# zzmuxi/simian-spacemonkey

Measured on AMD Instinct MI355X. Metric: Msamples/s + fps, 512^3 VGH vol @1024^2 x 512 steps, higher is better.
Workload: dtype f32

## Files before the change

simian-spacemonkey_amd/csrc/smk_api.hip:

```cpp
#include <math.h>
#include <stdio.h>
#include <string.h>

#include <algorithm>

#include "smk_device.h"

static std::string g_create_err;

#include <condition_variable>
#include <mutex>
#include <thread>
namespace {
struct HostPool {
  std::vector<std::thread> workers;
  std::mutex m, use;
  std::condition_variable cv, done_cv;
  const std::function<void(int)> *job = nullptr;
  int njobs = 0, next = 0, pending = 0;
  unsigned long long gen = 0;
  bool quit = false;
  explicit HostPool(int n) {
    for (int i = 0; i < n; ++i)
      workers.emplace_back([this] {
// ... 875 lines not shown
  for (int r = 0; r < c->nranks; ++r) {
    int key = 0;
    for (int bit = 0; bit < nbits; ++bit)
      if (((r >> bit) & 1) != nearbit[bit % 3]) key |= 1 << bit;
    keyed.push_back({key, r});
  }
  std::sort(keyed.begin(), keyed.end());
  for (int r = 0; r < c->nranks; ++r) order[r] = keyed[r].second;
}

extern "C" int smk_shard_order(smk_ctx *c, int *order) {
  if (!c || !order) return 1;
  if (!c->have_volume || !c->have_camera) FAIL(c, "smk_shard_order: volume and camera must be set");
  double inv[16];
  smk_inverse_affine(inv, c->mv);
  double e[3];
  for (int a = 0; a < 3; ++a) e[a] = inv[12 + a] * c->N[a] / c->fsize[a] - 0.5;
  smk_bsp_order(c, e, order);
  return 0;
}


extern "C" int smk_set_option(smk_ctx *c, const char *key, int value) {
  if (!c || !key) return 1;
  if (!strcmp(key, "kernel")) c->opt_kernel = value;
  else if (!strcmp(key, "slab_T")) c->slab.opt_T = value & 0xff;
  else if (!strcmp(key, "inject_slab_status")) c->opt_inject_status = value;
  else if (!strcmp(key, "slab_fly")) c->slab.opt_fly = value < 0 ? 0 : (value > 63 ? 63 : value);
  else if (!strcmp(key, "slab_ns")) c->slab.opt_ns = value < 0 ? 0 : (value > 63 ? 63 : value);
  else if (!strcmp(key, "tile")) c->slab.opt_tile = value;
  else if (!strcmp(key, "shadow_march")) c->opt_shadow_march = value ? 1 : 0;
  else if (!strcmp(key, "shadow_fused")) c->opt_lockstep = value ? (c->opt_lockstep | 256) : (c->opt_lockstep & ~256);
  else if (!strcmp(key, "slab_split")) c->slab.opt_split = value < 0 ? 0 : (value > 8 ? 8 : value);
  else if (!strcmp(key, "cols_shape")) c->cols.opt_shape = value & 0xff;
  else if (!strcmp(key, "cols_ns")) c->cols.opt_ns = value & 0xff;
  else if (!strcmp(key, "cols_chunk")) c->cols.opt_chunk = value & 0xfff;
  else if (!strcmp(key, "cols_wstep")) c->cols.opt_wstep = value & 7;
  else if (!strcmp(key, "cols_counts")) c->cols.want_counts = value ? 1 : 0;
  else if (!strcmp(key, "cols_fill")) { c->cols.opt_fill = value; smk_cols_drop_layouts(&c->cols); }
  else if (!strcmp(key, "cols_take_min")) c->cols.opt_take_min = value;
  else if (!strcmp(key, "cols_take_wait")) c->cols.opt_take_wait = value;
  else if (!strcmp(key, "cols_fly")) c->cols.opt_fly = value;
  else if (!strcmp(key, "bricks")) {
    c->opt_bricks = value ? 1 : 0;
    c->tf_dirty = true;
    c->bricks3_dirty = true;
  }
  else if (!strcmp(key, "wave_w")) {
    if (!(value == 1 || value == 2 || value == 4 || value == 8 || value == 16 || value == 32 || value == 64)) FAIL(c, "smk_set_option: wave_w must be a power of two <= 64");
    c->opt_wave_w = value;
  } else if (!strcmp(key, "blk_w")) {
    if (!(value == 1 || value == 2 || value == 4)) FAIL(c, "smk_set_option: blk_w must be 1, 2 or 4");
    c->opt_blk_w = value;
  } else if (!strcmp(key, "lockstep")) c->opt_lockstep = value;
  else if (!strcmp(key, "tf_raw")) {
    c->opt_tf_raw = value;
    c->tf_dirty = true;
  }
  else if (!strcmp(key, "halo")) {
    if (c->have_volume) FAIL(c, "smk_set_option: halo must be set before smk_upload_volume");
    if (value < 1) FAIL(c, "smk_set_option: halo must be >= 1");
    c->halo = value;
  } else
    FAIL(c, "smk_set_option: unknown key '%s'", key);
  return 0;
}
// ... 50 lines not shown
    return count_on_device(c, [&](unsigned long long *d) { return smk_launch_shadow_count_light(P, sc, olo, ohi, d, c->stream); }, value);
  }
  if (!strcmp(name, "slab_status")) {
    HIPCHK(c, hipDeviceSynchronize());
    *value = c->slab.h_status ? (((volatile int *)c->slab.h_status)[c->slab.status_slot] & 0xff) : 0;
    return 0;
  }
  if (!strcmp(name, "slab_failures")) {
    long long n = c->slab_failures;
    if (c->slab.h_status)
      for (int k = 0; k < SMK_STATUS_RING; ++k) n += ((volatile int *)c->slab.h_status)[k] != 0;
    *value = (double)n;
    return 0;
  }
  if (!strcmp(name, "slab_streamed_fraction")) {
    *value = 1.0;
    const int nt = c->slab.ticks_n_last;
    if (c->last_kernel == 2 && c->slab.d_ticks && nt > 0) {
      std::vector<unsigned> h((size_t)2 * nt);
      if (read_back(c, h.data(), c->slab.d_ticks + nt, h.size())) return 1;
      double st = 0, pl = 0;
      for (int t = 0; t < nt; ++t) {
        st += h[t];
        pl += h[(size_t)nt + t];
      }
      if (pl > 0) *value = st / pl;
    }
    return 0;
  }
  if (!strcmp(name, "slab_tile_ms_max") || !strcmp(name, "slab_tile_ms_sum")) {
    *value = 0.0;
    const int nt = c->slab.ticks_n_last;
    if (c->last_kernel == 2 && c->slab.d_ticks && nt > 0) {
      std::vector<unsigned> h((size_t)nt);
      if (read_back(c, h.data(), c->slab.d_ticks, h.size())) return 1;
      double mx = 0, sum = 0;
      for (int t = 0; t < nt; ++t) {
        const double k = t < (int)c->slab.ksplit_last.size() ? std::max<int>(c->slab.ksplit_last[t], 1) : 1;
        mx = std::max(mx, (double)h[t] / k);
        sum += h[t];
      }
      *value = (name[13] == 'm' ? mx : sum) * 1e-5;
    }
    return 0;
  }
  if (!strncmp(name, "cols_", 5)) return smk_cols_stat(c, name, value);
  if (!strcmp(name, "slab_split_tiles")) { *value = c->slab.nsplit_last; return 0; }
  if (!strcmp(name, "slab_workgroups")) { *value = c->slab.nblocks_last; return 0; }
  if (!strcmp(name, "slab_retries")) { *value = (double)c->slab_retries; return 0; }
  if (!strcmp(name, "clip_slice_pass")) { *value = c->clip_slice_pass; return 0; }
  FAIL(c, "smk_get_stat: unknown name '%s'", name);
}

extern "C" int smk_get_trace(smk_ctx *c, unsigned *out, int cap_records, int *nrecords) {
  if (!c || !nrecords) return 1;
  HIPCHK(c, hipSetDevice(c->device));
  if (!(c->opt_lockstep & 32)) {
    const int nt = c->last_kernel == 2 && c->slab.d_ticks ? c->slab.ticks_n_last : 0;
    *nrecords = nt;
    if (out && nt > 0) {
      std::vector<unsigned> h((size_t)nt * 5);
      if (read_back(c, h.data(), c->slab.d_ticks, h.size())) return 1;
      for (int t = 0; t < std::min(cap_records, nt); ++t) {
        unsigned *r = out + (size_t)t * 8;
        r[0] = h[(size_t)3 * nt + t];
        r[1] = h[(size_t)3 * nt + t] ? r[0] + h[t] : 0u;
        r[2] = h[(size_t)4 * nt + t] & 0xff00u;
        r[3] = (h[(size_t)4 * nt + t] & 0xfu) | ((unsigned)t << 8) | (h[(size_t)2 * nt + t] << 20);
        r[4] = r[5] = r[6] = r[7] = 0;
      }
    }
    return 0;
  }
  *nrecords = c->slab.d_trace ? c->slab.trace_n : 0;
  if (out && *nrecords > 0 && read_back(c, out, c->slab.d_trace, (size_t)std::min(cap_records, *nrecords) * 8)) return 1;
  return 0;
}

extern "C" int smk_count_samples(smk_ctx *c, double *in_volume) {
  if (!c || !in_volume) return 1;
  HIPCHK(c, hipSetDevice(c->device));
  RenderParams P;
  if (smk_build_params(c, P, c->stream)) return 1;
  smk_shadowcoef sc;
  if (c->shadow_on && c->tf_mode != 0 && !P.pert_on && !c->region_on && smk_shadow_setup(c, P, sc, nullptr, nullptr)) return 1;
  return count_on_device(c, [&](unsigned long long *d) { return smk_launch_count_inside(P, d, c->stream); }, in_volume);
}

void smk_region_box(const smk_ctx *c, const int g0[3], const int g1[3], float lo[3], float hi[3], int top[3]) {
  for (int a = 0; a < 3; ++a) {
    lo[a] = (float)g0[a] - 0.5f;
    hi[a] = (float)g1[a] - 0.5f;
    top[a] = g1[a] == c->N[a];
  }
  if (c->clip_axis >= 1 && c->clip_axis <= 6) {
    const int a = (c->clip_axis - 1) / 2;
    const float fs = c->fsize[a];
    const float cp = c->clip_vpos[a] > 0.0f ? (c->clip_vpos[a] < fs ? c->clip_vpos[a] : fs) : 0.0f;
    const float face = (float)((double)cp / (double)fs * (double)c->N[a] - 0.5);
// ... 357 lines not shown
```

simian-spacemonkey_amd/csrc/smk_internal.h:

```cpp
#pragma once
#include <hip/hip_runtime.h>
#include <stdint.h>

#include <map>
#include <string>
#include <vector>

#include "../../include/smk.h"

#define SMK_MAX_RANKS 8
#define SMK_TIMING_RING 64
#define SMK_BRICK_LOG2 3
#define SMK_SHADOW_BOX_EPS 0.0009765625f
#define SMK_TUNE_SETTLE 6
#define SMK_STATUS_RING 8

#define HIPCHK(ctx, call)                                                              \
  do {                                                                                 \
    hipError_t e_ = (call);                                                            \
    if (e_ != hipSuccess) {                                                            \
      char b_[512];                                                                    \
      snprintf(b_, sizeof b_, "%s failed: %s (%s:%d)", #call, hipGetErrorString(e_), __FILE__, __LINE__); \
      (ctx)->err = b_;                                                                 \
      return 1;                                                                        \
// ... 91 lines not shown
  std::vector<int2> order_host;
  struct Scan {
    std::vector<unsigned char> key;
    double v[4] = {0, 0, 0, 0};
    std::vector<int> work;
  } scan[4];
  unsigned scan_next = 0;
  std::vector<unsigned char> shape_key;
  int shape_choice = -1, shape_age = 0, shape_chunks = 0;
  std::vector<int> plan_work;
  std::vector<unsigned char> plan_cuts;
  std::vector<int2> plan_order;
  int plan_slots = 0;
  unsigned *d_ticks = nullptr, *h_ticks = nullptr;
  int ticks_cap = 0, ticks_pending_n = 0, ticks_age = 0, ticks_adopted = 0;
  int ticks_n_last = 0;
  bool ticks_pending = false;
  long long ticks_pending_sig = 0, ticks_good_sig = -1;
  hipEvent_t ticks_ev = nullptr;
  std::vector<unsigned> ticks_good;
  void *d_seg = nullptr;
  size_t seg_cap = 0;
  int opt_split = 0;
  int opt_tile = 0, opt_T = 0, opt_fly = 0, opt_ns = 0;
  bool ticks_stale = false;
  int nsplit_last = 0, nblocks_last = 0;
  std::vector<unsigned char> ksplit_last;
  unsigned *d_pticks = nullptr, *h_pticks = nullptr;
  std::vector<unsigned> pticks_good;
  std::vector<unsigned char> cuts, cuts_pending, cuts_good;
  int cuts_split = -1;
  long long cuts_sig = -1;
  bool recut = true, cuts_engaged = false, merge_warm = false;
  unsigned *d_trace = nullptr;
  int trace_cap = 0, trace_n = 0;
};

struct ColLayout {
  void *d = nullptr;
  size_t bytes = 0;
  int CW = 0, CH = 0, ncu = 0, ncv = 0, Du = 0, Dv = 0, Ds = 0, slice_bytes = 0, vb = 0;
  const void *src = nullptr;
};
struct ColsAux {
  ColLayout lay[3];
  void *d_layers = nullptr;
  size_t layers_cap = 0;
  void *d_masks = nullptr;
  size_t masks_cap = 0;
  bool masks_dirty = true;
  int mask_words_last = 0;
  unsigned *d_ticks = nullptr;
  int ticks_cap = 0, njobs_last = 0;
  unsigned long long *d_counts = nullptr;
  int want_counts = 0;
  int opt_shape = 0, opt_ns = 0, opt_chunk = 0, opt_wstep = 0;
  int opt_fill = 0, opt_take_min = 0, opt_take_wait = 0, opt_fly = 0;
  int builds = 0;
  int cw_last = 0, ch_last = 0, nslots_last = 0, shape_last = 0;
  double last_stream_bytes = 0;
  hipEvent_t frame_ev0 = nullptr;
  int status_tag = 0;
};
void smk_cols_free(ColsAux *aux);
void smk_cols_drop_layouts(ColsAux *aux);

// ... 240 lines not shown
```

simian-spacemonkey_amd/csrc/smk_slab.hip:

```cpp
#include <math.h>
#include <stdio.h>
#include <stdlib.h>
#include <string.h>

#include <algorithm>
#include <functional>
#include <type_traits>

#include "smk_device.h"
#include "smk_slab.h"

#define SLAB_DONE 0x3fffffff
constexpr int SLAB_POLL_SLEEP = 2;

template <int DT>
struct VoxT;
template <>
struct VoxT<0> {
  typedef uint2 type;
};
template <>
struct VoxT<1> {
  typedef float4 type;
};
// ... 93 lines not shown
  __builtin_memcpy(&lo, tb + off, 8);
  __builtin_memcpy(&hi, tb + (off + (unsigned)ss * 4u), 8);
  o.a = lo.x;
  o.b = lo.y;
  o.c = hi.x;
  o.d = hi.y;
  return o;
}
__device__ __forceinline__ float slab_tex_chan(const SlabTexel4 &x, int k) {
  return smk_lerp(smk_lerp(smk_ub(x.a, k), smk_ub(x.b, k), x.fs), smk_lerp(smk_ub(x.c, k), smk_ub(x.d, k), x.fs), x.ft) * SMK_INV255;
}

template <int DT, int SH, int PERM, int NW, int NL, bool DIAG, int TF = 1, bool BR = true, bool SHD = false, bool OCC = false>
__global__ __launch_bounds__((NW + NL) * 64, ((NW + NL) == 9) ? 6 : ((NW + NL) == 5 || (NW + NL) == 10) ? 5 : ((NW + NL) == 11 ? 3 : (NW + NL) == 12 ? 6 : 4)) void smk_k_slab(const RenderParams P, const SlabParams Q) {
  constexpr int UPV = DT == 0 ? 2 : 1;
  constexpr int VB = DT == 0 ? 8 : 16;
  constexpr int VBL = DT == 0 ? 3 : 4;
  constexpr int NTH = (NW + NL) * 64;
  constexpr bool BIG = slab_big(NW, NL);
  constexpr bool EARLY = BIG;
  constexpr bool FIFO = BIG;
  constexpr int NLG = slab_loader_groups(NW, NL);
  constexpr int LPG = NL / NLG;
  constexpr int QSTEP = NLG;
  extern __shared__ __align__(16) unsigned char smem[];
  SlabEnt *wtab = reinterpret_cast<SlabEnt *>(smem + (size_t)Q.nslots * Q.slot_bytes);
  int *ctl = reinterpret_cast<int *>(smem + (((size_t)Q.nslots * Q.slot_bytes + (size_t)Q.Ds * sizeof(SlabEnt) + 15) & ~(size_t)15));
  float *ah = reinterpret_cast<float *>(ctl + 8 + 32);
  const uint32_t *occ = reinterpret_cast<const uint32_t *>(ah + (Q.use_ah ? P.sv : 0));

  const int2 oent = Q.order[blockIdx.x];
  const int ocode = oent.x;
  if (ocode < 0) return;
  const int tile = ocode & 0xfffff, seg = (ocode >> 20) & 63, nseg = max((ocode >> 26) & 31, 1);
  const int cut_lo = oent.y & 255, cut_hi = (oent.y >> 8) & 255;
  const bool flags = BR && Q.bricks != nullptr;
  const bool tracing = DIAG && Q.trace != nullptr && (P.lockstep & 32);
  const unsigned trace_t0 = (unsigned)__builtin_amdgcn_s_memrealtime();
  const int ty = tile / P.ntx, tx = tile - ty * P.ntx;

  const int tid = threadIdx.x;
  const int lane = tid & 63;
  const int wave = __builtin_amdgcn_readfirstlane(tid >> 6);
  const bool is_loader = wave >= NW;
  const int lid = wave - NW;
  const int wpr = Q.tw >> 3;
  const int i = tx * Q.tw + (wave % wpr) * 8 + (lane & 7);
  const int j = ty * Q.th + (wave / wpr) * 8 + (lane >> 3);
  const bool live = !is_loader && i < P.W && j < P.H;

  const smk_raycoef &rc = P.rc;
  const float px = __fmaf_rn((float)i + 0.5f, rc.pxs, rc.pxl);
  const float py = __fmaf_rn((float)j + 0.5f, rc.pys, rc.pyl);
  float A[3], B[3], tauA, dtau;
  const bool ray_ok = smk_ray_AB_t<SHD>(P, px, py, A, B, tauA, dtau);
  float tenter = 0.0f, texit = (float)(rc.nplanes - 1);
  bool empty = rc.nplanes <= 0 || !live || !ray_ok;
#pragma unroll
  for (int a = 0; a < 3; ++a) {
    if (fabsf(B[a]) > 1e-20f) {
      float inv = 1.0f / B[a];
      float t1 = (P.lo[a] - SMK_RANGE_EPS - A[a]) * inv, t2 = (P.hi[a] + SMK_RANGE_EPS - A[a]) * inv;
      tenter = fmaxf(tenter, fminf(t1, t2) - 2.0f);
      texit = fminf(texit, fmaxf(t1, t2) + 2.0f);
    } else if (!(A[a] >= P.lo[a] && A[a] <= P.hi[a])) {
      empty = true;
    }
  }
  if (P.cplane_on) {
    const float c0 = __fmaf_rn(A[0], P.cplane[0], __fmaf_rn(A[1], P.cplane[1], __fmaf_rn(A[2], P.cplane[2], P.cplane[3])));
    const float c1 = __fmaf_rn(B[0], P.cplane[0], __fmaf_rn(B[1], P.cplane[1], B[2] * P.cplane[2]));
    if (fabsf(c1) > 1e-20f) {
      const float tz = -c0 / c1;
      if (c1 > 0.0f) tenter = fmaxf(tenter, tz - 2.0f);
      else texit = fminf(texit, tz + 2.0f);
    } else if (!(c0 >= 0.0f)) {
      empty = true;
    }
  }
  if (SHD && ray_ok) {
    if (fabsf(dtau) > 1e-30f) {
      const float tz = -tauA / dtau;
// ... 868 lines not shown
            car_i = base_slice_c(m, car_sc);
            pb = __mul24(psgn, car_i) + poff;
          } else pb = SLAB_DONE;
        }
        if (count) {
          n_it += 1.f;
          n_act += (float)__popcll(__ballot(act));
          n_in += (float)__popcll(__ballot(work));
          n_hit += (float)__popcll(__ballot(d_hit));
          n_anyhit += __any(d_hit) ? 1.f : 0.f;
          n_work += __any(work) ? 1.f : 0.f;
          n_own += __any(work && d_own) ? 1.f : 0.f;
        }
        }
      }
      if (lane == 0) lds_st(&ctl[8 + wave], SLAB_DONE);
      if (tracing && lane == 0) atomicAdd(Q.trace + 8 * (size_t)blockIdx.x + 7, (unsigned)n_it);
      if (count && lane == 0) {
        atomicAdd(&Q.diag[0], n_it);
        atomicAdd(&Q.diag[1], n_act);
        atomicAdd(&Q.diag[2], n_in);
        atomicAdd(&Q.diag[3], n_hit);
        atomicAdd(&Q.diag[8], n_anyhit);
        atomicAdd(&Q.diag[14], n_work);
        atomicAdd(&Q.diag[15], n_own);
        atomicAdd(&Q.diag[9], n_lead);
        atomicAdd(&Q.diag[10], n_waits);
        atomicAdd(&Q.diag[11], n_wstep);
        atomicAdd(&Q.diag[12], (float)max(npos - min(pos, npos), 0) / (float)max(npos, 1));
        atomicAdd(&Q.diag[13], 1.0f);
      }
    }
  }
  if (live) {
    size_t o = (size_t)j * P.W + i;
    float4 *outp = seg == 0 ? P.out : Q.seg_out + (size_t)(seg - 1) * ((size_t)P.W * P.H);
    outp[o] = make_float4(C0, C1, C2, C3);
    if (P.depth != nullptr && C3 == 0.0f) P.depth[o] = __int_as_float(0x7f800000);
  }
  if (npos > 0) {
    __syncthreads();
    if (tid == 0 && ctl[3]) *(volatile int *)Q.status = Q.status_tag | ctl[3];
  }
  if (tid == 0 && Q.tile_ticks && nseg > 1) {
    const unsigned dur = max((unsigned)__builtin_amdgcn_s_memrealtime() - trace_t0, 1u);
    if (Q.piece_ticks) Q.piece_ticks[(size_t)tile * 8 + seg] = dur;
    atomicAdd(&Q.tile_ticks[tile], dur);
    atomicAdd(&Q.tile_ticks[Q.ntiles + tile], npos > 0 ? (unsigned)max(min(max(min(min(ctl[4], ctl[5]), min(ctl[6], ctl[7])), 0), npos + 1) - ctl[2], 0) : 0u);
    atomicAdd(&Q.tile_ticks[2 * Q.ntiles + tile], npos > 0 ? (unsigned)(npos + 1) : 0u);
  } else if (tid == 0 && Q.tile_ticks) {
    Q.tile_ticks[tile] = max((unsigned)__builtin_amdgcn_s_memrealtime() - trace_t0, 1u);
    Q.tile_ticks[Q.ntiles + tile] = npos > 0 ? (unsigned)max(min(max(min(min(ctl[4], ctl[5]), min(ctl[6], ctl[7])), 0), npos + 1) - ctl[2], 0) : 0u;
    Q.tile_ticks[2 * Q.ntiles + tile] = npos > 0 ? (unsigned)(npos + 1) : 0u;
    Q.tile_ticks[3 * Q.ntiles + tile] = trace_t0;
    Q.tile_ticks[4 * Q.ntiles + tile] = (__builtin_amdgcn_s_getreg((31 << 11) | 4) & 0xff00u) | (__builtin_amdgcn_s_getreg((31 << 11) | 20) & 0xfu);
  }
  if (tracing && tid == 0) {
    unsigned *t = Q.trace + 8 * (size_t)blockIdx.x;
    if (phases) {
      t[4] = ph1;
      t[5] = ph2;
      t[6] = ph3;
    }
    t[0] = trace_t0;
    t[1] = (unsigned)__builtin_amdgcn_s_memrealtime();
    t[2] = __builtin_amdgcn_s_getreg((31 << 11) | 4);
    t[3] = (__builtin_amdgcn_s_getreg((31 << 11) | 20) & 0xf) | ((unsigned)tile << 8) | ((unsigned)max(npos, 0) << 20);
  }
}


#ifndef SLAB_PART
#define SLAB_PART 0
#endif
#if SLAB_PART == 0
__global__ __launch_bounds__(256) void smk_k_slab_merge(const int2 *list, int tw, int th, int ntx, int W, int H, const float4 *seg_out, float4 *out, int use_max) {
  const int code = list[blockIdx.x].x;
  const int tile = code & 0xfffff, nseg = code >> 20;
  const int ty = tile / ntx, tx = tile - ty * ntx;
  const size_t npix = (size_t)W * H;
  for (int p = threadIdx.x; p < tw * th; p += blockDim.x) {
    const int i = tx * tw + p % tw, j = ty * th + p / tw;
    if (i >= W || j >= H) continue;
    const size_t o = (size_t)j * W + i;
    float4 C = out[o];
    for (int k = 1; k < nseg; ++k) {
      const float4 sgm = seg_out[(size_t)(k - 1) * npix + o];
      if (use_max) {
        C = make_float4(fmaxf(C.x, sgm.x), fmaxf(C.y, sgm.y), fmaxf(C.z, sgm.z), fmaxf(C.w, sgm.w));
      } else {
        const float w = 1.0f - C.w;
        C.x = __fmaf_rn(w, sgm.x, C.x);
        C.y = __fmaf_rn(w, sgm.y, C.y);
        C.z = __fmaf_rn(w, sgm.z, C.z);
        C.w = __fmaf_rn(w, sgm.w, C.w);
      }
    }
    out[o] = C;
  }
}
// ... 130 lines not shown
```

simian-spacemonkey_amd/csrc/smk_slab_plan.hip:

```cpp
#include <math.h>
#include <stdio.h>
#include <stdlib.h>
#include <string.h>
#include <time.h>

#include <algorithm>
#include <vector>

#include "smk_slab.h"

void host_ray_at(const RenderParams &P, double px, double py, double A[3], double B[3]) {
  const smk_raycoef &rc = P.rc;
  if (!P.sh.on) {
    for (int a = 0; a < 3; ++a) {
      A[a] = px * rc.Ax[a] + py * rc.Ay[a] + rc.Ac[a];
      B[a] = px * rc.Bx[a] + py * rc.By[a] + rc.Bc[a];
    }
    return;
  }
  const SmkShadowRays &sh = P.sh;
  const double nD = px * sh.nDx + py * sh.nDy + sh.nDc, tauA = sh.numA / nD, dtau = sh.dB / nD;
  for (int a = 0; a < 3; ++a) {
    const double D = px * sh.Dx[a] + py * sh.Dy[a] + sh.Dc[a];
    A[a] = sh.Ec[a] + tauA * D;
// ... 530 lines not shown
    if (aux->h_pticks) (void)hipHostFree(aux->h_pticks);
    aux->d_ticks = aux->h_ticks = aux->d_pticks = aux->h_pticks = nullptr;
    aux->ticks_cap = 0;
    hipError_t e = hipMalloc((void **)&aux->d_ticks, (size_t)nt * 20);
    if (e == hipSuccess) e = hipMemset(aux->d_ticks, 0, (size_t)nt * 20);
    if (e == hipSuccess) e = hipHostMalloc((void **)&aux->h_ticks, (size_t)nt * 4, hipHostMallocDefault);
    if (e == hipSuccess) e = hipMalloc((void **)&aux->d_pticks, (size_t)nt * 32);
    if (e == hipSuccess) e = hipMemset(aux->d_pticks, 0, (size_t)nt * 32);
    if (e == hipSuccess) e = hipHostMalloc((void **)&aux->h_pticks, (size_t)nt * 32, hipHostMallocDefault);
    if (e != hipSuccess) return e;
    aux->ticks_cap = nt;
  }
  if (!aux->ticks_ev) {
    hipError_t e = hipEventCreateWithFlags(&aux->ticks_ev, hipEventDisableTiming);
    if (e != hipSuccess) return e;
  }
  Q.tile_ticks = aux->d_ticks;
  Q.piece_ticks = aux->d_pticks;
  Q.ntiles = nt;
  aux->ticks_n_last = nt;
  return hipSuccess;
}

void smk_slab_forget_measurements(SlabAux *aux) {
  aux->ticks_good.clear();
  aux->ticks_good_sig = -1;
  aux->ticks_adopted = 0;
  aux->ticks_stale = aux->ticks_pending;
  aux->pticks_good.clear();
  aux->cuts_good.clear();
  aux->cuts.clear();
  aux->cuts_sig = -1;
  aux->cuts_engaged = false;
  aux->recut = true;
}

void smk_slab_free(SlabAux *aux) {
  for (void *p : {(void *)aux->d_diag, (void *)aux->d_order, (void *)aux->d_pticks, aux->d_seg, (void *)aux->d_trace, (void *)aux->d_ticks})
    if (p) (void)hipFree(p);
  for (void *p : {(void *)aux->h_status, (void *)aux->h_pticks, (void *)aux->h_ticks, (void *)aux->h_order[0], (void *)aux->h_order[1],
                  (void *)aux->h_order[2], (void *)aux->h_order[3]})
    if (p) (void)hipHostFree(p);
  for (hipEvent_t e : {aux->order_ev[0], aux->order_ev[1], aux->order_ev[2], aux->order_ev[3], aux->ticks_ev})
    if (e) (void)hipEventDestroy(e);
}

static void slab_cut_segments(SlabAux *aux, const std::vector<int> &work, int nt, long long tsig, int opt_split, bool big) {
  const bool measured = aux->ticks_good_sig == tsig && (int)aux->ticks_good.size() == nt;
  if ((int)aux->cuts.size() != nt * 10 || aux->cuts_split != opt_split || aux->cuts_sig != tsig) {
    aux->cuts.assign((size_t)nt * 10, 0);
    for (int t = 0; t < nt; ++t) { aux->cuts[(size_t)t * 10] = 1; aux->cuts[(size_t)t * 10 + 2] = 255; }
    aux->cuts_split = opt_split;
    aux->cuts_sig = tsig;
    aux->recut = true;
  }
  if (aux->recut) {
    aux->recut = false;
    auto equal_cuts = [&](int t, int K) {
      unsigned char *c = &aux->cuts[(size_t)t * 10];
      c[0] = (unsigned char)K;
      for (int k = 0; k <= K; ++k) c[1 + k] = (unsigned char)(255 * k / K);
    };
    if (opt_split >= 2) {
      for (int t = 0; t < nt; ++t) equal_cuts(t, std::min(opt_split, 8));
    } else if (opt_split == 0 && measured) {
      long long total = 0;
      for (int t = 0; t < nt; ++t) total += work[t];
      const double wg_slots = 256.0 * (big ? 1 : 2);
      const double mean_load = (double)total / wg_slots;
      double longest_tile = 0;
      for (int t = 0; t < nt; ++t) longest_tile = std::max(longest_tile, (double)work[t]);
      const double piece = std::max(0.75 * mean_load, 6000.0);
      bool big_frame = mean_load >= 5000.0 && longest_tile > 1.5 * mean_load;
      if (aux->cuts_engaged && mean_load >= 5000.0 && longest_tile > 1.2 * mean_load) big_frame = true;
      aux->cuts_engaged = big_frame;
      const bool have_pieces = (int)aux->pticks_good.size() == nt * 8 && (int)aux->cuts_good.size() == nt * 10;
      for (int t = 0; t < nt; ++t) {
        unsigned char *c = &aux->cuts[(size_t)t * 10];
        int Kw = (big_frame && (double)work[t] > 1.25 * piece) ? (int)std::min(8.0, ceil((double)work[t] / piece)) : 1;
        if (big_frame && c[0] >= 2 && Kw >= 1 && abs(Kw - (int)c[0]) <= 1 && (double)work[t] > piece) Kw = c[0];
        if (Kw == 1) { equal_cuts(t, 1); continue; }
        const unsigned char *g = have_pieces ? &aux->cuts_good[(size_t)t * 10] : nullptr;
        const int Kg = g ? g[0] : 1;
        if (!g || Kg < 2) {
          if (c[0] != Kw) equal_cuts(t, Kw);
          continue;
        }
        double d[8], tot = 0, longest = 0;
        for (int k = 0; k < Kg; ++k) {
          d[k] = std::max(1.0, (double)aux->pticks_good[(size_t)t * 8 + k] - 1300.0);
          tot += d[k];
          longest = std::max(longest, d[k]);
        }
        const bool same = !memcmp(g, c, 10);
        if (same && Kg == Kw && longest <= 1.3 * tot / Kg) continue;
        unsigned char nc[10] = {(unsigned char)Kw, 0};
        int k = 0;
        double acc = 0;
        for (int j = 1; j < Kw; ++j) {
          const double want = tot * j / Kw;
          while (k < Kg - 1 && acc + d[k] < want) acc += d[k++];
          const double f = d[k] > 0 ? (want - acc) / d[k] : 0.5;
          int x = (int)lround(g[1 + k] + f * (g[2 + k] - g[1 + k]));
          x = std::max(x, (int)nc[j] + 1);
          x = std::min(x, 255 - (Kw - j));
          nc[1 + j] = (unsigned char)x;
        }
        nc[1 + Kw] = 255;
        memcpy(c, nc, 10);
      }
    } else {
      for (int t = 0; t < nt; ++t) equal_cuts(t, 1);
    }
  }
}

static void slab_schedule(const RenderParams &P, SlabAux *aux, const std::vector<int> &work, int slots, std::vector<int2> &order) {
  const int nt = P.ntx * P.nty;
  if (aux->plan_slots == slots && aux->plan_work == work && aux->plan_cuts == aux->cuts && !aux->plan_order.empty()) {
    order = aux->plan_order;
    return;
  }
  std::vector<unsigned char> ksplit((size_t)nt, 1);
  for (int t = 0; t < nt; ++t) ksplit[t] = aux->cuts[(size_t)t * 10];
  auto piece_weight = [&](int t, int k) -> int {
    const unsigned char *c = &aux->cuts[(size_t)t * 10];
    if ((int)aux->pticks_good.size() == nt * 8 && (int)aux->cuts_good.size() == nt * 10 && !memcmp(&aux->cuts_good[(size_t)t * 10], c, 10) &&
        aux->pticks_good[(size_t)t * 8 + k] > 0)
      return (int)std::min<unsigned>(aux->pticks_good[(size_t)t * 8 + k], 1u << 30);
    return work[t] / std::max<int>(c[0], 1);
  };
  std::vector<std::vector<int>> run(8);
  std::vector<int> ws;
  ws.reserve((size_t)nt);
  for (int t = 0; t < nt; ++t)
    if (work[t] > 0) ws.push_back(work[t]);
  std::sort(ws.begin(), ws.end());
  const bool even = ws.size() >= 16 && (long long)ws[ws.size() * 95 / 100] * 4 <= (long long)ws[ws.size() / 2] * 5;
  const int SLAB_DEAL_W = even ? 4 : 2, SLAB_DEAL_H = even ? 4 : 2;
  const int gbx = (P.ntx + SLAB_DEAL_W - 1) / SLAB_DEAL_W, gby = (P.nty + SLAB_DEAL_H - 1) / SLAB_DEAL_H;
  std::vector<long long> gw((size_t)gbx * gby, 0);
  for (int t = 0; t < nt; ++t) gw[(size_t)((t / P.ntx) / SLAB_DEAL_H) * gbx + (t % P.ntx) / SLAB_DEAL_W] += work[t];
  std::vector<int> idx((size_t)gbx * gby);
  for (int g = 0; g < gbx * gby; ++g) idx[g] = g;
  std::stable_sort(idx.begin(), idx.end(), [&](int a, int b) { return gw[a] > gw[b]; });
  long long load[8] = {0, 0, 0, 0, 0, 0, 0, 0};
  for (int g : idx) {
    int x = 0;
    for (int k = 1; k < 8; ++k)
      if (load[k] < load[x]) x = k;
    const int gy = g / gbx, gx = g - gy * gbx;
    for (int dy = 0; dy < SLAB_DEAL_H; ++dy)
      for (int dx = 0; dx < SLAB_DEAL_W; ++dx) {
        const int ty = gy * SLAB_DEAL_H + dy, tx = gx * SLAB_DEAL_W + dx;
        if (ty < P.nty && tx < P.ntx) run[x].push_back(ty * P.ntx + tx);
      }
    load[x] += gw[g];
  }
  for (int x = 0; x < 8; ++x)
    std::stable_sort(run[x].begin(), run[x].end(), [&](int a, int b) { return work[a] / ksplit[a] > work[b] / ksplit[b]; });
  size_t longest = 0;
  std::vector<std::vector<std::pair<int, int2>>> items(8);
  for (int x = 0; x < 8; ++x) {
    for (int t : run[x]) {
      const unsigned char *c = &aux->cuts[(size_t)t * 10];
      for (int k = 0; k < c[0]; ++k)
        items[x].push_back({piece_weight(t, k), make_int2(t | (k << 20) | ((int)c[0] << 26), (int)c[1 + k] | ((int)c[2 + k] << 8))});
    }
    std::stable_sort(items[x].begin(), items[x].end(), [](const std::pair<int, int2> &a, const std::pair<int, int2> &b) { return a.first > b.first; });
    longest = std::max(longest, items[x].size());
  }
  order.assign(longest * 8, make_int2(-1, 0));
  for (int x = 0; x < 8; ++x)
    for (size_t k = 0; k < items[x].size(); ++k) order[k * 8 + x] = items[x][k].second;
  int nsplit = 0;
  for (int t = 0; t < nt; ++t)
    if (ksplit[t] > 1) { order.push_back(make_int2(t | ((int)ksplit[t] << 20), 0)); ++nsplit; }
  order.push_back(make_int2(nsplit, 0));
  aux->plan_work = work;
  aux->plan_cuts = aux->cuts;
  aux->plan_order = order;
  aux->plan_slots = slots;
}

static hipError_t slab_segments(const RenderParams &P, SlabParams &Q, SlabAux *aux, const std::vector<int2> &order, int *nblocks) {
  const int nt = P.ntx * P.nty;
  const int nsplit = order.back().x;
  *nblocks = (int)order.size() - 1 - nsplit;
  aux->ksplit_last.assign((size_t)nt, 1);
  int maxseg = 1;
  for (int k = 0; k < nsplit; ++k) {
    const int code = order[(size_t)*nblocks + k].x;
    aux->ksplit_last[code & 0xfffff] = (unsigned char)(code >> 20);
    maxseg = std::max(maxseg, code >> 20);
  }
  aux->nsplit_last = nsplit;
  aux->nblocks_last = *nblocks;
  if (maxseg > 1) {
    const size_t need = (size_t)(8 - 1) * P.W * P.H * 16;
    if (need > aux->seg_cap) {
      if (aux->d_seg) (void)hipFree(aux->d_seg);
      aux->d_seg = nullptr;
      aux->seg_cap = 0;
      hipError_t e = hipMalloc(&aux->d_seg, need);
      if (e != hipSuccess) return e;
      aux->seg_cap = need;
    }
  }
  Q.seg_out = (float4 *)aux->d_seg;
  return hipSuccess;
}

static hipError_t slab_upload_order(SlabAux *aux, std::vector<int2> &order, hipStream_t s) {
  if (aux->frame_ev0) {
    hipError_t e = hipEventRecord(aux->frame_ev0, s);
    if (e != hipSuccess) return e;
  }
  auto same_order = [&]() { return aux->order_host.size() == order.size() && (order.empty() || !memcmp(aux->order_host.data(), order.data(), order.size() * sizeof(int2))); };
  if (!same_order()) {
    if ((int)order.size() > aux->order_cap) {
      if (aux->d_order) (void)hipFree(aux->d_order);
      aux->d_order = nullptr;
      for (int k = 0; k < 4; ++k) {
        if (aux->order_ev[k]) (void)hipEventSynchronize(aux->order_ev[k]);
        if (aux->h_order[k]) (void)hipHostFree(aux->h_order[k]);
        aux->h_order[k] = nullptr;
      }
      aux->order_cap = 0;
      const size_t cap = order.size() * 2 + 1024;
      hipError_t e = hipMalloc((void **)&aux->d_order, cap * sizeof(int2));
// ... 7 lines not shown
    if (e != hipSuccess) return e;
    memcpy(aux->h_order[k], order.data(), order.size() * sizeof(int2));
    e = hipMemcpyAsync(aux->d_order, aux->h_order[k], order.size() * sizeof(int2), hipMemcpyHostToDevice, s);
    if (e != hipSuccess) return e;
    e = hipEventRecord(aux->order_ev[k], s);
    if (e != hipSuccess) return e;
    aux->order_host.swap(order);
  }
  return hipSuccess;
}

static hipError_t slab_trace(const RenderParams &P, SlabParams &Q, SlabAux *aux, int nblocks, hipStream_t s) {
  Q.trace = nullptr;
  if (!(P.lockstep & 32)) return hipSuccess;
  if (nblocks > aux->trace_cap) {
    if (aux->d_trace) (void)hipFree(aux->d_trace);
    aux->d_trace = nullptr;
    aux->trace_cap = 0;
    hipError_t e = hipMalloc((void **)&aux->d_trace, (size_t)nblocks * 32);
    if (e != hipSuccess) return e;
    aux->trace_cap = nblocks;
  }
  hipError_t e = hipMemsetAsync(aux->d_trace, 0, (size_t)nblocks * 32, s);
  if (e != hipSuccess) return e;
  aux->trace_n = nblocks;
  Q.trace = aux->d_trace;
  return hipSuccess;
}

static hipError_t slab_run(const RenderParams &P, const SlabParams &Q, SlabAux *aux, int dtype, int tf_mode, int shade_kind, SlabShape sh,
                           size_t lds, int nblocks, long long tsig, const char **why, hipStream_t s) {
  const int nw = slab_waves(sh), nt = Q.ntiles, nsplit = aux->nsplit_last;
  const bool diag = (P.lockstep & ~1) != 0 && dtype == 1 && shade_kind == 1;
  hipError_t e = nsplit > 0 ? hipMemsetAsync(aux->d_ticks, 0, (size_t)nt * 20, s) : hipSuccess;
  if (e != hipSuccess) return e;
  if (!aux->merge_warm && nblocks >= 1) {
    aux->merge_warm = true;
    static const int2 one = make_int2(0 | (1 << 20), 0);
    int2 *d_one = nullptr;
    if (hipMalloc((void **)&d_one, sizeof one) == hipSuccess) {
      if (hipMemcpyAsync(d_one, &one, sizeof one, hipMemcpyHostToDevice, s) == hipSuccess)
        (void)smk_slab_merge(d_one, 1, sh.tw, sh.th, P.ntx, P.W, P.H, (const float4 *)P.out, P.out, 0, s);
      (void)hipStreamSynchronize(s);
      (void)hipFree(d_one);
    }
    (void)hipGetLastError();
  }
  e = P.zscene   ? (P.sh.on ? smk_slab_dispatch_occluded_shadow(P, Q, dtype, tf_mode, shade_kind, nw, sh.nl, lds, nblocks, why, s)
                             : smk_slab_dispatch_occluded(P, Q, dtype, tf_mode, shade_kind, nw, sh.nl, lds, nblocks, why, s))
      : P.sh.on    ? smk_slab_dispatch_shadow(P, Q, dtype, tf_mode, shade_kind, nw, sh.nl, lds, nblocks, why, s)
      : dtype == 0 ? smk_slab_dispatch_u8(P, Q, tf_mode, shade_kind, nw, sh.nl, diag, lds, nblocks, why, s)
                   : smk_slab_dispatch_f32(P, Q, tf_mode, shade_kind, nw, sh.nl, diag, lds, nblocks, why, s);
  if (e == hipSuccess && nsplit > 0)
    e = smk_slab_merge(aux->d_order + nblocks, nsplit, sh.tw, sh.th, P.ntx, P.W, P.H, (const float4 *)aux->d_seg, P.out,
                       P.blend == SMK_BLEND_MAX ? 1 : 0, s);
  if (e != hipSuccess || aux->ticks_pending) return e;
  e = hipMemcpyAsync(aux->h_ticks, aux->d_ticks, (size_t)nt * 4, hipMemcpyDeviceToHost, s);
  if (e == hipSuccess && nsplit > 0) e = hipMemcpyAsync(aux->h_pticks, aux->d_pticks, (size_t)nt * 32, hipMemcpyDeviceToHost, s);
  if (nsplit > 0) aux->cuts_pending = aux->cuts; else aux->cuts_pending.clear();
  if (e == hipSuccess) e = hipEventRecord(aux->ticks_ev, s);
  if (e != hipSuccess) return e;
  aux->ticks_pending = true;
  aux->ticks_pending_sig = tsig;
  aux->ticks_pending_n = nt;
  return hipSuccess;
}

static hipError_t slab_plan_and_launch(RenderParams &P, int dtype, int tf_mode, int shade_kind, const void *vox_native, const void *vox_xmajor,
                                       SlabAux *aux, const char **why, hipStream_t s) {
  const double t0 = slab_clock.on ? slab_now() : 0;
  slab_clock.frame_scan = 0;
  SlabParams Q;
  memset(&Q, 0, sizeof Q);
  Q.status = aux->h_status + aux->status_slot;
  Q.status_tag = aux->status_tag;
  Q.diag = aux->d_diag;
  const double ds = slab_axes(P, vox_native, vox_xmajor, Q);
  if ((*why = slab_refusal(P, dtype, tf_mode, Q))) return hipErrorNotSupported;
  if (tf_mode == 0) shade_kind = 0;
  SlabShape shape;
  size_t lds = 0;
  std::vector<int> work;
  if ((*why = slab_choose_shape(P, Q, dtype, tf_mode, ds, aux, shape, &lds, work))) return hipErrorNotSupported;

  const int nw = slab_waves(shape), nt = P.ntx * P.nty;
  const long long tsig = (((long long)P.ntx * 4096 + P.nty) * 64 + shape.tw) * 64 + shape.th + ((long long)(Q.perm * 2 + (Q.dir > 0)) << 48) +
                         ((long long)nw << 52) + ((long long)dtype << 56);
  hipError_t e = slab_measured_weights(aux, tsig, nt, work, Q);
  if (e != hipSuccess) return e;
  const int opt_split = P.depth ? 1 : aux->opt_split;
  slab_cut_segments(aux, work, nt, tsig, opt_split, slab_big(nw, shape.nl));
  std::vector<int2> order;
  slab_schedule(P, aux, work, (nw + shape.nl) | (opt_split << 12), order);
  int nblocks = 0;
  if ((e = slab_segments(P, Q, aux, order, &nblocks)) != hipSuccess) return e;
  if (slab_clock.on) {
    slab_clock.scan += slab_clock.frame_scan;
    slab_clock.planned += slab_now() - t0;
    if (++slab_clock.n % 60 == 0) {
      fprintf(stderr, "[smk] planning per frame: scans %.3f ms, all of it up to the launch %.3f ms, whole launcher (previous 60) %.3f ms\n",
              slab_clock.scan / 60, slab_clock.planned / 60, slab_clock.whole / 60);
      slab_clock.scan = slab_clock.planned = slab_clock.whole = 0;
    }
  }
  if ((e = slab_upload_order(aux, order, s)) != hipSuccess) return e;
  Q.order = aux->d_order;
  if ((e = slab_trace(P, Q, aux, nblocks, s)) != hipSuccess) return e;
  return slab_run(P, Q, aux, dtype, tf_mode, shade_kind, shape, lds, nblocks, tsig, why, s);
}

hipError_t smk_launch_slab(RenderParams P, int dtype, int tf_mode, int shade_kind, const void *vox_native, const void *vox_xmajor, SlabAux *aux,
                           const char **why, hipStream_t s) {
  const double t0 = slab_clock.on ? slab_now() : 0;
  const hipError_t e = slab_plan_and_launch(P, dtype, tf_mode, shade_kind, vox_native, vox_xmajor, aux, why, s);
  if (slab_clock.on) slab_clock.whole += slab_now() - t0;
  return e;
}
```

Baseline: 936,400.

## Split heavy slab tiles laterally across wave subsets to balance workgroup load

Adds lateral splitting of heavy tiles: a tile is launched as several workgroups, and each one uses only a subset of the waves, selected by a wave mask packed into the order entry. The planner picks the split factor from measured per-tile work, by default up to 2 pieces for tiles much heavier than the mean workgroup load. This is meant to shorten the longest-tile tail of the dispatch. In exchange, more workgroups re-stream the same slab data with fewer active waves, and the order-code bit layout changes, which reduces the maximum segment count to 8.

```diff
diff --git a/simian-spacemonkey_amd/csrc/smk_api.hip b/simian-spacemonkey_amd/csrc/smk_api.hip
--- a/simian-spacemonkey_amd/csrc/smk_api.hip
+++ b/simian-spacemonkey_amd/csrc/smk_api.hip
@@ -931,6 +931,8 @@
   else if (!strcmp(key, "shadow_march")) c->opt_shadow_march = value ? 1 : 0;
   else if (!strcmp(key, "shadow_fused")) c->opt_lockstep = value ? (c->opt_lockstep | 256) : (c->opt_lockstep & ~256);
   else if (!strcmp(key, "slab_split")) c->slab.opt_split = value < 0 ? 0 : (value > 8 ? 8 : value);
+  else if (!strcmp(key, "slab_lateral")) c->slab.opt_lateral = value < 0 ? 0 : (value > 16 ? 16 : value);
+  else if (!strcmp(key, "slab_lateral_share")) { c->slab.opt_lat_share = value < 0 ? 0 : value; c->slab.lat_opt = -1; }
   else if (!strcmp(key, "cols_shape")) c->cols.opt_shape = value & 0xff;
   else if (!strcmp(key, "cols_ns")) c->cols.opt_ns = value & 0xff;
   else if (!strcmp(key, "cols_chunk")) c->cols.opt_chunk = value & 0xfff;
@@ -1047,12 +1049,22 @@
     *value = 0.0;
     const int nt = c->slab.ticks_n_last;
     if (c->last_kernel == 2 && c->slab.d_ticks && nt > 0) {
-      std::vector<unsigned> h((size_t)nt);
+      std::vector<unsigned> h((size_t)nt), hp;
       if (read_back(c, h.data(), c->slab.d_ticks, h.size())) return 1;
+      if (c->slab.nlat_last > 0 && c->slab.d_pticks) {
+        hp.resize((size_t)nt * 8);
+        if (read_back(c, hp.data(), c->slab.d_pticks, hp.size())) return 1;
+      }
       double mx = 0, sum = 0;
       for (int t = 0; t < nt; ++t) {
-        const double k = t < (int)c->slab.ksplit_last.size() ? std::max<int>(c->slab.ksplit_last[t], 1) : 1;
-        mx = std::max(mx, (double)h[t] / k);
+        const int k = t < (int)c->slab.ksplit_last.size() ? std::max<int>(c->slab.ksplit_last[t], 1) : 1;
+        const int l = t < (int)c->slab.lat_last.size() ? std::max<int>(c->slab.lat_last[t], 1) : 1;
+        double longest = (double)h[t] / (k * l);
+        if (k == 1 && l > 1 && l <= 8 && !hp.empty()) {
+          longest = 0;
+          for (int p = 0; p < l; ++p) longest = std::max(longest, (double)hp[(size_t)t * 8 + p]);
+        }
+        mx = std::max(mx, longest);
         sum += h[t];
       }
       *value = (name[13] == 'm' ? mx : sum) * 1e-5;
@@ -1061,6 +1073,7 @@
   }
   if (!strncmp(name, "cols_", 5)) return smk_cols_stat(c, name, value);
   if (!strcmp(name, "slab_split_tiles")) { *value = c->slab.nsplit_last; return 0; }
+  if (!strcmp(name, "slab_lateral_tiles")) { *value = c->slab.nlat_last; return 0; }
   if (!strcmp(name, "slab_workgroups")) { *value = c->slab.nblocks_last; return 0; }
   if (!strcmp(name, "slab_retries")) { *value = (double)c->slab_retries; return 0; }
   if (!strcmp(name, "clip_slice_pass")) { *value = c->clip_slice_pass; return 0; }
@@ -1074,12 +1087,18 @@
     const int nt = c->last_kernel == 2 && c->slab.d_ticks ? c->slab.ticks_n_last : 0;
     *nrecords = nt;
     if (out && nt > 0) {
-      std::vector<unsigned> h((size_t)nt * 5);
+      std::vector<unsigned> h((size_t)nt * 5), hp;
       if (read_back(c, h.data(), c->slab.d_ticks, h.size())) return 1;
+      if ((c->slab.nlat_last > 0 || c->slab.nsplit_last > 0) && c->slab.d_pticks) {
+        hp.resize((size_t)nt * 8);
+        if (read_back(c, hp.data(), c->slab.d_pticks, hp.size())) return 1;
+      }
       for (int t = 0; t < std::min(cap_records, nt); ++t) {
         unsigned *r = out + (size_t)t * 8;
+        const bool in_pieces = !hp.empty() && ((t < (int)c->slab.ksplit_last.size() && c->slab.ksplit_last[t] > 1) ||
+                                               (t < (int)c->slab.lat_last.size() && c->slab.lat_last[t] > 1));
         r[0] = h[(size_t)3 * nt + t];
-        r[1] = h[(size_t)3 * nt + t] ? r[0] + h[t] : 0u;
+        r[1] = h[(size_t)3 * nt + t] ? r[0] + (in_pieces ? hp[(size_t)t * 8] : h[t]) : 0u;
         r[2] = h[(size_t)4 * nt + t] & 0xff00u;
         r[3] = (h[(size_t)4 * nt + t] & 0xfu) | ((unsigned)t << 8) | (h[(size_t)2 * nt + t] << 20);
         r[4] = r[5] = r[6] = r[7] = 0;
diff --git a/simian-spacemonkey_amd/csrc/smk_internal.h b/simian-spacemonkey_amd/csrc/smk_internal.h
--- a/simian-spacemonkey_amd/csrc/smk_internal.h
+++ b/simian-spacemonkey_amd/csrc/smk_internal.h
@@ -147,6 +147,11 @@
   int cuts_split = -1;
   long long cuts_sig = -1;
   bool recut = true, cuts_engaged = false, merge_warm = false;
+  std::vector<unsigned char> lat, plan_lat, lat_last;
+  int opt_lateral = 0;
+  int opt_lat_share = 0;
+  int lat_opt = -1, nlat_last = 0;
+  long long lat_sig = -1;
   unsigned *d_trace = nullptr;
   int trace_cap = 0, trace_n = 0;
 };
diff --git a/simian-spacemonkey_amd/csrc/smk_slab.hip b/simian-spacemonkey_amd/csrc/smk_slab.hip
--- a/simian-spacemonkey_amd/csrc/smk_slab.hip
+++ b/simian-spacemonkey_amd/csrc/smk_slab.hip
@@ -149,8 +149,9 @@
   const int2 oent = Q.order[blockIdx.x];
   const int ocode = oent.x;
   if (ocode < 0) return;
-  const int tile = ocode & 0xfffff, seg = (ocode >> 20) & 63, nseg = max((ocode >> 26) & 31, 1);
+  const int tile = ocode & 0xfffff, seg = (ocode >> 20) & 7, nseg = max((ocode >> 26) & 15, 1);
   const int cut_lo = oent.y & 255, cut_hi = (oent.y >> 8) & 255;
+  const unsigned wmask = (unsigned)oent.y >> 16;
   const bool flags = BR && Q.bricks != nullptr;
   const bool tracing = DIAG && Q.trace != nullptr && (P.lockstep & 32);
   const unsigned trace_t0 = (unsigned)__builtin_amdgcn_s_memrealtime();
@@ -164,7 +165,7 @@
   const int wpr = Q.tw >> 3;
   const int i = tx * Q.tw + (wave % wpr) * 8 + (lane & 7);
   const int j = ty * Q.th + (wave / wpr) * 8 + (lane >> 3);
-  const bool live = !is_loader && i < P.W && j < P.H;
+  const bool live = !is_loader && ((wmask >> wave) & 1u) && i < P.W && j < P.H;
 
   const smk_raycoef &rc = P.rc;
   const float px = __fmaf_rn((float)i + 0.5f, rc.pxs, rc.pxl);
@@ -1099,9 +1100,13 @@
       }
     }
   }
+  int ocode_e = ocode;
+  asm volatile("" : "+s"(ocode_e));
+  const int tile_e = ocode_e & 0xfffff, seg_e = (ocode_e >> 20) & 7, lat_k = (ocode_e >> 23) & 7;
+  const int pieces_e = (ocode_e >> 26) & 31;
   if (live) {
     size_t o = (size_t)j * P.W + i;
-    float4 *outp = seg == 0 ? P.out : Q.seg_out + (size_t)(seg - 1) * ((size_t)P.W * P.H);
+    float4 *outp = seg_e == 0 ? P.out : Q.seg_out + (size_t)(seg_e - 1) * ((size_t)P.W * P.H);
     outp[o] = make_float4(C0, C1, C2, C3);
     if (P.depth != nullptr && C3 == 0.0f) P.depth[o] = __int_as_float(0x7f800000);
   }
@@ -1109,18 +1114,22 @@
     __syncthreads();
     if (tid == 0 && ctl[3]) *(volatile int *)Q.status = Q.status_tag | ctl[3];
   }
-  if (tid == 0 && Q.tile_ticks && nseg > 1) {
+  if (tid == 0 && Q.tile_ticks && pieces_e > 1) {
     const unsigned dur = max((unsigned)__builtin_amdgcn_s_memrealtime() - trace_t0, 1u);
-    if (Q.piece_ticks) Q.piece_ticks[(size_t)tile * 8 + seg] = dur;
-    atomicAdd(&Q.tile_ticks[tile], dur);
-    atomicAdd(&Q.tile_ticks[Q.ntiles + tile], npos > 0 ? (unsigned)max(min(max(min(min(ctl[4], ctl[5]), min(ctl[6], ctl[7])), 0), npos + 1) - ctl[2], 0) : 0u);
-    atomicAdd(&Q.tile_ticks[2 * Q.ntiles + tile], npos > 0 ? (unsigned)(npos + 1) : 0u);
+    if (Q.piece_ticks && ((pieces_e & 15) <= 1 || lat_k == 0)) Q.piece_ticks[(size_t)tile_e * 8 + (seg_e | lat_k)] = dur;
+    if (seg_e == 0 && lat_k == 0) {
+      Q.tile_ticks[3 * Q.ntiles + tile_e] = trace_t0;
+      Q.tile_ticks[4 * Q.ntiles + tile_e] = (__builtin_amdgcn_s_getreg((31 << 11) | 4) & 0xff00u) | (__builtin_amdgcn_s_getreg((31 << 11) | 20) & 0xfu);
+    }
+    atomicAdd(&Q.tile_ticks[tile_e], dur);
+    atomicAdd(&Q.tile_ticks[Q.ntiles + tile_e], npos > 0 ? (unsigned)max(min(max(min(min(ctl[4], ctl[5]), min(ctl[6], ctl[7])), 0), npos + 1) - ctl[2], 0) : 0u);
+    atomicAdd(&Q.tile_ticks[2 * Q.ntiles + tile_e], npos > 0 ? (unsigned)(npos + 1) : 0u);
   } else if (tid == 0 && Q.tile_ticks) {
-    Q.tile_ticks[tile] = max((unsigned)__builtin_amdgcn_s_memrealtime() - trace_t0, 1u);
-    Q.tile_ticks[Q.ntiles + tile] = npos > 0 ? (unsigned)max(min(max(min(min(ctl[4], ctl[5]), min(ctl[6], ctl[7])), 0), npos + 1) - ctl[2], 0) : 0u;
-    Q.tile_ticks[2 * Q.ntiles + tile] = npos > 0 ? (unsigned)(npos + 1) : 0u;
-    Q.tile_ticks[3 * Q.ntiles + tile] = trace_t0;
-    Q.tile_ticks[4 * Q.ntiles + tile] = (__builtin_amdgcn_s_getreg((31 << 11) | 4) & 0xff00u) | (__builtin_amdgcn_s_getreg((31 << 11) | 20) & 0xfu);
+    Q.tile_ticks[tile_e] = max((unsigned)__builtin_amdgcn_s_memrealtime() - trace_t0, 1u);
+    Q.tile_ticks[Q.ntiles + tile_e] = npos > 0 ? (unsigned)max(min(max(min(min(ctl[4], ctl[5]), min(ctl[6], ctl[7])), 0), npos + 1) - ctl[2], 0) : 0u;
+    Q.tile_ticks[2 * Q.ntiles + tile_e] = npos > 0 ? (unsigned)(npos + 1) : 0u;
+    Q.tile_ticks[3 * Q.ntiles + tile_e] = trace_t0;
+    Q.tile_ticks[4 * Q.ntiles + tile_e] = (__builtin_amdgcn_s_getreg((31 << 11) | 4) & 0xff00u) | (__builtin_amdgcn_s_getreg((31 << 11) | 20) & 0xfu);
   }
   if (tracing && tid == 0) {
     unsigned *t = Q.trace + 8 * (size_t)blockIdx.x;
@@ -1132,7 +1141,7 @@
     t[0] = trace_t0;
     t[1] = (unsigned)__builtin_amdgcn_s_memrealtime();
     t[2] = __builtin_amdgcn_s_getreg((31 << 11) | 4);
-    t[3] = (__builtin_amdgcn_s_getreg((31 << 11) | 20) & 0xf) | ((unsigned)tile << 8) | ((unsigned)max(npos, 0) << 20);
+    t[3] = (__builtin_amdgcn_s_getreg((31 << 11) | 20) & 0xf) | ((unsigned)tile_e << 8) | ((unsigned)max(npos, 0) << 20);
   }
 }
 
diff --git a/simian-spacemonkey_amd/csrc/smk_slab_plan.hip b/simian-spacemonkey_amd/csrc/smk_slab_plan.hip
--- a/simian-spacemonkey_amd/csrc/smk_slab_plan.hip
+++ b/simian-spacemonkey_amd/csrc/smk_slab_plan.hip
@@ -586,6 +586,8 @@
   aux->cuts.clear();
   aux->cuts_sig = -1;
   aux->cuts_engaged = false;
+  aux->lat.clear();
+  aux->lat_sig = -1;
   aux->recut = true;
 }
 
@@ -599,7 +601,7 @@
     if (e) (void)hipEventDestroy(e);
 }
 
-static void slab_cut_segments(SlabAux *aux, const std::vector<int> &work, int nt, long long tsig, int opt_split, bool big) {
+static bool slab_cut_segments(SlabAux *aux, const std::vector<int> &work, int nt, long long tsig, int opt_split, bool big) {
   const bool measured = aux->ticks_good_sig == tsig && (int)aux->ticks_good.size() == nt;
   if ((int)aux->cuts.size() != nt * 10 || aux->cuts_split != opt_split || aux->cuts_sig != tsig) {
     aux->cuts.assign((size_t)nt * 10, 0);
@@ -608,6 +610,7 @@
     aux->cuts_sig = tsig;
     aux->recut = true;
   }
+  const bool recut = aux->recut;
   if (aux->recut) {
     aux->recut = false;
     auto equal_cuts = [&](int t, int K) {
@@ -623,7 +626,8 @@
       const double wg_slots = 256.0 * (big ? 1 : 2);
       const double mean_load = (double)total / wg_slots;
       double longest_tile = 0;
-      for (int t = 0; t < nt; ++t) longest_tile = std::max(longest_tile, (double)work[t]);
+      const bool lat_known = (int)aux->lat.size() == nt;
+      for (int t = 0; t < nt; ++t) longest_tile = std::max(longest_tile, (double)work[t] / (lat_known ? std::max<int>(aux->lat[t], 1) : 1));
       const double piece = std::max(0.75 * mean_load, 6000.0);
       bool big_frame = mean_load >= 5000.0 && longest_tile > 1.5 * mean_load;
       if (aux->cuts_engaged && mean_load >= 5000.0 && longest_tile > 1.2 * mean_load) big_frame = true;
@@ -667,16 +671,49 @@
       for (int t = 0; t < nt; ++t) equal_cuts(t, 1);
     }
   }
-}
-
-static void slab_schedule(const RenderParams &P, SlabAux *aux, const std::vector<int> &work, int slots, std::vector<int2> &order) {
+  return recut;
+}
+
+constexpr double SLAB_LATERAL_SHARE = 1.0;
+constexpr int SLAB_LATERAL_MOST = 2;
+static void slab_cut_lateral(SlabAux *aux, const std::vector<int> &work, int nt, long long tsig, int opt_lateral, int nw, bool big, bool recut) {
+  const bool measured = aux->ticks_good_sig == tsig && (int)aux->ticks_good.size() == nt;
+  if ((int)aux->lat.size() != nt || aux->lat_opt != opt_lateral || aux->lat_sig != tsig) {
+    aux->lat.assign((size_t)nt, 1);
+    aux->lat_opt = opt_lateral;
+    aux->lat_sig = tsig;
+    recut = true;
+  }
+  if (!recut) return;
+  if (opt_lateral >= 2) {
+    std::fill(aux->lat.begin(), aux->lat.end(), (unsigned char)std::min(opt_lateral, nw));
+  } else if (opt_lateral == 0 && measured) {
+    long long total = 0;
+    for (int t = 0; t < nt; ++t) total += work[t];
+    const double mean_load = (double)total / (256.0 * (big ? 1 : 2));
+    const double share = aux->opt_lat_share > 0 ? aux->opt_lat_share * 0.01 : SLAB_LATERAL_SHARE;
+    const double piece = std::max(share * mean_load, 6000.0);
+    for (int t = 0; t < nt; ++t) {
+      const bool may = mean_load >= 5000.0 && aux->cuts[(size_t)t * 10] == 1;
+      int Lw = (may && (double)work[t] > 1.25 * piece) ? (int)std::min((double)std::min(nw, SLAB_LATERAL_MOST), ceil((double)work[t] / piece)) : 1;
+      const int L = aux->lat[t];
+      if (may && L >= 2 && abs(Lw - L) <= 1 && (double)work[t] > piece) Lw = L;
+      aux->lat[t] = (unsigned char)Lw;
+    }
+  } else {
+    std::fill(aux->lat.begin(), aux->lat.end(), (unsigned char)1);
+  }
+}
+
+static void slab_schedule(const RenderParams &P, SlabAux *aux, const std::vector<int> &work, int slots, int nw, std::vector<int2> &order) {
   const int nt = P.ntx * P.nty;
-  if (aux->plan_slots == slots && aux->plan_work == work && aux->plan_cuts == aux->cuts && !aux->plan_order.empty()) {
+  if (aux->plan_slots == slots && aux->plan_work == work && aux->plan_cuts == aux->cuts && aux->plan_lat == aux->lat && !aux->plan_order.empty()) {
     order = aux->plan_order;
     return;
   }
   std::vector<unsigned char> ksplit((size_t)nt, 1);
   for (int t = 0; t < nt; ++t) ksplit[t] = aux->cuts[(size_t)t * 10];
+  auto pieces = [&](int t) -> int { return (int)ksplit[t] * std::max<int>(aux->lat[t], 1); };
   auto piece_weight = [&](int t, int k) -> int {
     const unsigned char *c = &aux->cuts[(size_t)t * 10];
     if ((int)aux->pticks_good.size() == nt * 8 && (int)aux->cuts_good.size() == nt * 10 && !memcmp(&aux->cuts_good[(size_t)t * 10], c, 10) &&
@@ -712,14 +749,19 @@
     load[x] += gw[g];
   }
   for (int x = 0; x < 8; ++x)
-    std::stable_sort(run[x].begin(), run[x].end(), [&](int a, int b) { return work[a] / ksplit[a] > work[b] / ksplit[b]; });
+    std::stable_sort(run[x].begin(), run[x].end(), [&](int a, int b) { return work[a] / pieces(a) > work[b] / pieces(b); });
   size_t longest = 0;
   std::vector<std::vector<std::pair<int, int2>>> items(8);
   for (int x = 0; x < 8; ++x) {
     for (int t : run[x]) {
       const unsigned char *c = &aux->cuts[(size_t)t * 10];
+      const int L = std::max<int>(aux->lat[t], 1);
       for (int k = 0; k < c[0]; ++k)
-        items[x].push_back({piece_weight(t, k), make_int2(t | (k << 20) | ((int)c[0] << 26), (int)c[1 + k] | ((int)c[2 + k] << 8))});
+        for (int l = 0; l < L; ++l) {
+          const unsigned waves = ((1u << ((l + 1) * nw / L)) - (1u << (l * nw / L))) << 16;
+          const int piece = L > 1 ? (std::min(l, 7) << 23) | (1 << 30) : 0;
+          items[x].push_back({piece_weight(t, k) / L, make_int2(t | (k << 20) | ((int)c[0] << 26) | piece, (int)((unsigned)c[1 + k] | ((unsigned)c[2 + k] << 8) | waves))});
+        }
     }
     std::stable_sort(items[x].begin(), items[x].end(), [](const std::pair<int, int2> &a, const std::pair<int, int2> &b) { return a.first > b.first; });
     longest = std::max(longest, items[x].size());
@@ -733,6 +775,7 @@
   order.push_back(make_int2(nsplit, 0));
   aux->plan_work = work;
   aux->plan_cuts = aux->cuts;
+  aux->plan_lat = aux->lat;
   aux->plan_order = order;
   aux->plan_slots = slots;
 }
@@ -750,6 +793,8 @@
   }
   aux->nsplit_last = nsplit;
   aux->nblocks_last = *nblocks;
+  aux->lat_last = aux->lat;
+  aux->nlat_last = (int)std::count_if(aux->lat.begin(), aux->lat.end(), [](unsigned char l) { return l > 1; });
   if (maxseg > 1) {
     const size_t need = (size_t)(8 - 1) * P.W * P.H * 16;
     if (need > aux->seg_cap) {
@@ -823,7 +868,7 @@
                            size_t lds, int nblocks, long long tsig, const char **why, hipStream_t s) {
   const int nw = slab_waves(sh), nt = Q.ntiles, nsplit = aux->nsplit_last;
   const bool diag = (P.lockstep & ~1) != 0 && dtype == 1 && shade_kind == 1;
-  hipError_t e = nsplit > 0 ? hipMemsetAsync(aux->d_ticks, 0, (size_t)nt * 20, s) : hipSuccess;
+  hipError_t e = nsplit > 0 || aux->nlat_last > 0 ? hipMemsetAsync(aux->d_ticks, 0, (size_t)nt * 20, s) : hipSuccess;
   if (e != hipSuccess) return e;
   if (!aux->merge_warm && nblocks >= 1) {
     aux->merge_warm = true;
@@ -880,9 +925,10 @@
   hipError_t e = slab_measured_weights(aux, tsig, nt, work, Q);
   if (e != hipSuccess) return e;
   const int opt_split = P.depth ? 1 : aux->opt_split;
-  slab_cut_segments(aux, work, nt, tsig, opt_split, slab_big(nw, shape.nl));
+  const bool recut = slab_cut_segments(aux, work, nt, tsig, opt_split, slab_big(nw, shape.nl));
+  slab_cut_lateral(aux, work, nt, tsig, aux->opt_lateral, nw, slab_big(nw, shape.nl), recut);
   std::vector<int2> order;
-  slab_schedule(P, aux, work, (nw + shape.nl) | (opt_split << 12), order);
+  slab_schedule(P, aux, work, (nw + shape.nl) | (opt_split << 12) | (aux->opt_lateral << 16), nw, order);
   int nblocks = 0;
   if ((e = slab_segments(P, Q, aux, order, &nblocks)) != hipSuccess) return e;
   if (slab_clock.on) {
```

Result: no change. 943,700, median of 2 (+0.8%).
